# ut-amrl/IV_SLAM

Measured on AMD Instinct MI355X. Metric: stereo pairs/s (extract+match+introspect) @1242×375, 1000 feat; 1/2/4/8 GPU, higher is better.
Workload: dtype u8 (ORB) + f32 via split-f16 MFMA (FCN)

## Files before the change

### iv_slam_amd/csrc/ivf_device.h

```cpp
#pragma once
#include <hip/hip_runtime.h>
#include <stdint.h>
#include <stdlib.h>
#include <vector>
#include "../../include/ivfront.h"

#define DEVINL __device__ __forceinline__

namespace ivf {

constexpr int kMaxLevels = IVF_MAX_LEVELS;
constexpr int kMaxCells = 2048;
constexpr int kEdge = 19;

struct LevelGeom {
    int w, h, pitch;
    int off;
    int nDesired;
    int cols, rows, cellW, cellH, nCells, nfeaturesCell;
    int maxBX, maxBY;
    int domH[2];
    int domHLast;
    int winHLast;
    int cellBase;
    int candBase, candCap;
    int kpBase;
    int scaledPatch;
    int tileBase, tilesX, tilesY;
    int btileBase, btilesX, btilesY;
    int rtX, rtY;
    int valid;
    float scale;
    unsigned cellWMagic, cellHMagic;
};

struct Config {
    int nlevels, w, h;
    int nfeatures, iniTh, minTh, introspection;
    int pyrBytes;
    int candTotal;
    int nCellsTotal;
    int nTiles;
    int nBlurTiles;
    int varBlur, varRetain, varAtan;
    int maxCandCap;
    int umax[16];
    float scale[kMaxLevels], invScale[kMaxLevels];
    int cellBases[kMaxLevels];
    int tileBases[kMaxLevels], btileBases[kMaxLevels];
    LevelGeom lv[kMaxLevels];
};

typedef unsigned long long ResizeCoef;

void resize_axis_table(int ssize, int dsize, int32_t* idx0, int32_t* idx1, int16_t* w0, int16_t* w1);
void resize_axis_pack(int ssize, int dsize, bool columns, bool withIdx1, std::vector<ResizeCoef>& tab);

struct UndistortCam { double fx, fy, cx, cy, k[12]; };
inline UndistortCam undistort_cam(const ivf_camera& c)
{
    UndistortCam u{};
    u.fx = (double)c.fx; u.fy = (double)c.fy; u.cx = (double)c.cx; u.cy = (double)c.cy;
    for (int i = 0; i < 12; i++) u.k[i] = i < c.n_dist ? (double)c.dist[i] : 0.;
    return u;
}
__host__ __device__ inline void undistort_point(const UndistortCam& c, float px, float py, float& ox, float& oy)
{
    const double* k = c.k;
    const double ifx = 1. / c.fx, ify = 1. / c.fy;
    const double u = (double)px, v = (double)py;
    double x = (u - c.cx) * ifx, y = (v - c.cy) * ify;
    const double x0 = x, y0 = y;
    for (int j = 0; j < 5; j++) {
        const double r2 = x * x + y * y;
        const double icdist = (1 + ((k[7] * r2 + k[6]) * r2 + k[5]) * r2) / (1 + ((k[4] * r2 + k[1]) * r2 + k[0]) * r2);
        if (icdist < 0) { x = (u - c.cx) * ifx; y = (v - c.cy) * ify; break; }
        const double dX = 2 * k[2] * x * y + k[3] * (r2 + 2 * x * x) + k[8] * r2 + k[9] * r2 * r2;
        const double dY = k[2] * (r2 + 2 * y * y) + 2 * k[3] * x * y + k[10] * r2 + k[11] * r2 * r2;
        x = (x0 - dX) * icdist; y = (y0 - dY) * icdist;
    }
    const double xx = c.fx * x + 0. * y + c.cx, yy = 0. * x + c.fy * y + c.cy, ww = 1. / (0. * x + 0. * y + 1.);
    ox = (float)(xx * ww); oy = (float)(yy * ww);
}

#ifndef IVF_FAST_TH
#define IVF_FAST_TH 32
#endif
constexpr int kFastTW = 128, kFastTH = IVF_FAST_TH;
constexpr int kBlurTW = 128, kBlurTH = 32;
constexpr int kTileCap = kFastTW * kFastTH / 4;
constexpr int kRowCap = 96;
constexpr int kHugeSlots = 8;
constexpr int kHugeListCap = 4096;

struct CellInfo { int nTotal, nRetain, prefix, useMin; };

struct Buffers {
    uint8_t* pyr;
    uint8_t* qpyr;
    uint8_t* blur;
    unsigned* tileList;
    int* tileCnt;
    int* cellCnt;
    unsigned long long* lvl;
    CellInfo* cellInfo;
    int* lvlTotal;
    unsigned int* slotPos;
    float* slotResp;
    int* lvlCount;
    uint8_t* useCost;
    ivf_keypoint* kps;
    uint8_t* desc;
    int* count;
    float* quality;
    float* uright;
    float* depth;
    int* sad;
    int* rowCnt;
    unsigned short* rowList;
    int* status;
    int* hugeCount;
    int* tierList;
    int* hugeList;
    unsigned* hugeScratch;
};

struct StereoArgs {
    const uint8_t *pyrL, *pyrR; size_t pyrStride;
    const ivf_keypoint *kpL, *kpR; const uint8_t *descL, *descR; const int *cntL, *cntR;
    size_t kpStride;
    int cntStride;
    float *uright, *depth; int* sad; int outStride;
    float bf, bb;
    int* rowCnt; unsigned short* rowList;
};

#ifdef IVF_EXPERIMENT
#define IVF_EXP_ENV(name) getenv(name)
#else
#define IVF_EXP_ENV(name) ((const char*)nullptr)
#endif

void count_launch();
}
#undef hipLaunchKernelGGL
#define hipLaunchKernelGGL(kernelName, ...) do { ivf::count_launch(); hipLaunchKernelGGLInternal((kernelName), __VA_ARGS__); } while (0)
namespace ivf {

int set_error(int code, const char* fmt, ...);

int thread_scratch(int device, size_t need, uint8_t** out);
int thread_pinned(size_t need, uint8_t** out);
int have_device(int dev);

struct BatchImage { const ivf_keypoint *kps, *mvKeys; const uint8_t* desc; const float *uright, *depth, *quality; const int* count; int cap; hipEvent_t done; };
int frame_from_batch(int device, const BatchImage& src, const ivf_bounds& bounds, ivf_frame** out);

void launch_stereo_args(const Config& hc, const Config* dc, const StereoArgs& A, int nPairs, hipStream_t s);
void launch_ingest(const Config& hc, const Config* dc, const uint8_t* src0, const uint8_t* src1, size_t imageStride, int rowStride,
                   int nImg, int nSides, uint8_t* dstBlob, const uint8_t* onlyFlagged, hipStream_t s, int sideMask = 3);
void launch_ingest_color(const Config& hc, const Config* dc, const uint8_t* src, size_t imageStride, int rowStride, int code, int nImg, int nSides, int side,
                         uint8_t* dstBlob, hipStream_t s);
void launch_pyramid(const Config& hc, const Config* dc, const ResizeCoef* dTab, uint8_t* blob, uint8_t* qblob, const uint8_t* useCost,
                    int nImg, hipStream_t s);
void launch_fast(const Config& hc, const Config* dc, const Buffers& b, int nImg, hipStream_t s);
void launch_blur(const Config& hc, const Config* dc, const Buffers& b, int nImg, hipStream_t s, bool skipEmptyLevels);
void launch_describe(const Config& hc, const Config* dc, const Buffers& b, int nImg, hipStream_t s);
void launch_stereo(const Config& hc, const Config* dc, const Buffers& b, int nPairs, float bf, float bb, hipStream_t s);
void launch_pack_gather(const Buffers& b, const ivf_keypoint* kpsUn, int nf, int nPairs, uint8_t* block, size_t recBytes, hipStream_t s);
void launch_select(const Config& hc, const Config* dc, const Buffers& b, int nImg, hipStream_t s);
void launch_test_retain_best(const float* dResp, int n, int nPoints, int* dOrder, unsigned long long* dLists, int* dDiffer, hipStream_t s);
void launch_undistort_keys(const UndistortCam& cam, bool passThrough, const ivf_keypoint* kps, size_t kpStride, const int* count, int cntStride,
                           int nFrames, int cap, ivf_keypoint* out, size_t outStride, hipStream_t s);
// ... 87 lines not shown
```

### iv_slam_amd/csrc/ivf_kernels.hip

```cpp
#include "ivf_grid.h"
#include <cstdlib>

namespace ivf {

static __device__ const int8_t __attribute__((aligned(16))) d_pattern[1024] = {
#include "../../include/ivf_pattern31.inc"
};

DEVINL bool xcd_tile_image(int nTiles, int nImg, int& tile, int& img)
{
    const int xcd = blockIdx.x & 7, j = blockIdx.x >> 3;
    img = (j / nTiles) * 8 + xcd; tile = j % nTiles;
    return img < nImg;
}

constexpr int kIngestRows = 8;
__global__ __launch_bounds__(256) void k_ingest(const Config* __restrict__ cfg, const uint8_t* __restrict__ src0,
                                               const uint8_t* __restrict__ src1, size_t imageStride, int rowStride, int nSides,
                                               uint8_t* __restrict__ blob, const uint8_t* __restrict__ onlyFlagged, int sideMask)
{
    const LevelGeom& G = cfg->lv[0];
    const int img = blockIdx.y, y0 = blockIdx.x * kIngestRows;
    if (onlyFlagged && !(use_cost_of(onlyFlagged, img) & 3u)) return;
    if (!((sideMask >> (img % nSides)) & 1)) return;
// ... 152 lines not shown
        for (int rr = 0; rr < kPyrRPT; rr++) {
            const ResizeCoef c = ty[min(dyFirst + rr, D.h - 1)];
            cyl[rr] = (unsigned)c; cyh[rr] = (unsigned)(c >> 32);
        }
#pragma unroll
        for (int rr = 0; rr < kPyrRPT; rr++) asm volatile("" : "+s"(cyl[rr]), "+s"(cyh[rr]));
#pragma unroll
        for (int rr = 0; rr < kPyrRPT; rr++) {
            const int dy = dyFirst + rr;
            if (dy >= D.h) break;
            const ResizeCoef cy = (ResizeCoef)cyl[rr] | ((ResizeCoef)cyh[rr] << 32);
            const int y0 = (int)(cy & 0xffff), y1 = min(y0 + 1, S.h - 1);
            const unsigned b0 = (unsigned)((cy >> 16) & 0xffff), b1 = (unsigned)((cy >> 32) & 0xffff);
            if (y0 - wy0 == rowB) {
#pragma unroll
                for (int k = 0; k < 4; k++) hA[k] = hB[k];
                rowA = rowB;
            } else if (y0 - wy0 != rowA) { hpass(y0 - wy0, hA); rowA = y0 - wy0; }
            if (y1 - wy0 == rowA) {
#pragma unroll
                for (int k = 0; k < 4; k++) hB[k] = hA[k];
                rowB = rowA;
            } else if (y1 - wy0 != rowB) { hpass(y1 - wy0, hB); rowB = y1 - wy0; }
            unsigned out = 0;
#pragma unroll
            for (int k = 0; k < 4; k++)
                out |= (((__umul24(b0, hA[k]) >> 16) + (__umul24(b1, hB[k]) >> 16) + 2u) >> 2) << (8 * k);
            *(unsigned*)(outp + (size_t)rr * D.pitch) = out & colMask;
        }
        return;
    }
    const int x4 = dx0 + (tid & 63) * 4;
    if (x4 >= D.pitch) return;
    int sxk[4], sx1k[4], a0k[4], a1k[4];
#pragma unroll
    for (int k = 0; k < 4; k++) {
        const int dx = min(x4 + k, D.w - 1);
        const ResizeCoef cx = tx[dx];
        sxk[k] = (int)(cx & 0xffff); sx1k[k] = min(sxk[k] + 1, S.w - 1);
        a0k[k] = (int)((cx >> 16) & 0xffff); a1k[k] = (int)((cx >> 32) & 0xffff);
    }
    for (int rr = 0; rr < kPyrTH / 4; rr++) {
        const int dy = dy0 + (tid >> 6) + 4 * rr;
        if (dy >= D.h) break;
        const ResizeCoef cy = ty[dy];
        const int y0 = (int)(cy & 0xffff), y1 = min(y0 + 1, S.h - 1);
        const int b0 = (int)((cy >> 16) & 0xffff), b1 = (int)((cy >> 32) & 0xffff);
        unsigned out = 0;
#pragma unroll
        for (int k = 0; k < 4; k++) {
            unsigned r = 0;
            if (x4 + k < D.w) {
                int p00, p01, p10, p11;
                const uint8_t* r0 = SP + (size_t)y0 * S.pitch;
                const uint8_t* r1 = SP + (size_t)y1 * S.pitch;
                p00 = r0[sxk[k]]; p01 = r0[sx1k[k]]; p10 = r1[sxk[k]]; p11 = r1[sx1k[k]];
                const int h0 = p00 * a0k[k] + p01 * a1k[k], h1 = p10 * a0k[k] + p11 * a1k[k];
                r = (unsigned)((((b0 * (h0 >> 4)) >> 16) + ((b1 * (h1 >> 4)) >> 16) + 2) >> 2) & 0xffu;
            }
            out |= r << (8 * k);
        }
        *(unsigned*)(base + D.off + (size_t)dy * D.pitch + x4) = out;
    }
}

__global__ __launch_bounds__(256) void k_pyr_down(const Config* __restrict__ cfg, int level, const ResizeCoef* __restrict__ tab,
                                                 uint8_t* __restrict__ blobI, uint8_t* __restrict__ blobQ,
                                                 const uint8_t* __restrict__ useCost, int nImg, int ldsPitch, int ldsRows)
{
    extern __shared__ __attribute__((aligned(16))) uint8_t src[];
    int img = blockIdx.z;
    uint8_t* blob = blobI;
    if (img >= nImg) { img -= nImg; blob = blobQ; if (!(use_cost_of(useCost, img) & 1u)) return; }
    pyr_tile(cfg, level, tab, blob + (size_t)img * cfg->pyrBytes, blockIdx.x * kPyrTW, blockIdx.y * kPyrTH, ldsPitch, ldsRows, src);
}

typedef short s16x2 __attribute__((ext_vector_type(2)));
DEVINL s16x2 pkmin(s16x2 a, s16x2 b) { return __builtin_elementwise_min(a, b); }
DEVINL s16x2 pkmax(s16x2 a, s16x2 b) { return __builtin_elementwise_max(a, b); }
DEVINL s16x2 pair_at(unsigned lo, unsigned hi, int i)
{
    return __builtin_bit_cast(s16x2, __builtin_amdgcn_perm(hi, lo, 0x0c000c00u | ((unsigned)(i + 1) << 16) | (unsigned)i));
}
DEVINL bool compass_test(s16x2 v, s16x2 p0, s16x2 p8, s16x2 p4, s16x2 p12, int t)
{
    const s16x2 T = {(short)t, (short)t};
    const s16x2 X = pkmax(pkmin(p0, p8), pkmin(p4, p12)), Y = pkmin(pkmax(p0, p8), pkmax(p4, p12));
    return ((__builtin_bit_cast(unsigned, X - (v - T)) | __builtin_bit_cast(unsigned, (v + T) - Y)) & 0x80008000u) != 0u;
}
DEVINL bool fast_precheck_pair(unsigned loT, unsigned hiT, unsigned loC, unsigned hiC, unsigned loB, unsigned hiB, int t)
{
    const s16x2 v = pair_at(loC, hiC, 3);
    return compass_test(v, pair_at(loB, hiB, 3), pair_at(loT, hiT, 3), pair_at(loC, hiC, 6), pair_at(loC, hiC, 0), t);
}
DEVINL bool fast_precheck_pair_b(unsigned t0, unsigned t1, unsigned m0, unsigned m1, unsigned m2, unsigned b0, unsigned b1, int t)
{
    const s16x2 v = pair_at(m0, m1, 5);
    return compass_test(v, pair_at(b0, b1, 5), pair_at(t0, t1, 5), pair_at(m1, m2, 4), pair_at(m0, m1, 2), t);
}
DEVINL unsigned fast_score_pair(const unsigned (&lo)[7], const unsigned (&hi)[7], int t)
{
    const s16x2 v = pair_at(lo[3], hi[3], 3);
    s16x2 p[16];
    p[0] = pair_at(lo[6], hi[6], 3);   p[1] = pair_at(lo[6], hi[6], 4);   p[2] = pair_at(lo[5], hi[5], 5);
    p[3] = pair_at(lo[4], hi[4], 6);   p[4] = pair_at(lo[3], hi[3], 6);   p[5] = pair_at(lo[2], hi[2], 6);
    p[6] = pair_at(lo[1], hi[1], 5);   p[7] = pair_at(lo[0], hi[0], 4);   p[8] = pair_at(lo[0], hi[0], 3);
    p[9] = pair_at(lo[0], hi[0], 2);   p[10] = pair_at(lo[1], hi[1], 1);  p[11] = pair_at(lo[2], hi[2], 0);
    p[12] = pair_at(lo[3], hi[3], 0);  p[13] = pair_at(lo[4], hi[4], 0);  p[14] = pair_at(lo[5], hi[5], 1);
    p[15] = pair_at(lo[6], hi[6], 2);
    s16x2 X = pkmin(p[0], p[8]), Y = pkmax(p[0], p[8]);
#pragma unroll
    for (int k = 1; k < 8; k++) { X = pkmax(X, pkmin(p[k], p[k + 8])); Y = pkmin(Y, pkmax(p[k], p[k + 8])); }
    const s16x2 T = {(short)t, (short)t};
    const s16x2 u = X - (v - T), w = (v + T) - Y;
    if (((__builtin_bit_cast(unsigned, u) | __builtin_bit_cast(unsigned, w)) & 0x80008000u) == 0u) return 0u;
    const s16x2 sg = (w >> 15) | (s16x2){1, 1};
    s16x2 q[16];
#pragma unroll
    for (int k = 0; k < 16; k++) q[k] = p[k] * sg;
    s16x2 mx[8];
#pragma unroll
    for (int i = 0; i < 8; i++) { const int j = 2 * i + 1; mx[i] = pkmax(q[j], q[(j + 1) & 15]); }
    s16x2 m4[8];
#pragma unroll
    for (int i = 0; i < 8; i++) m4[i] = pkmax(mx[i], mx[(i + 1) & 7]);
    s16x2 wmin;
#pragma unroll
    for (int i = 0; i < 8; i++) {
        const int j = 2 * i + 1;
        const s16x2 w8 = pkmax(m4[i], m4[(i + 2) & 7]);
        const s16x2 a = pkmax(w8, pkmin(q[(j + 15) & 15], q[(j + 8) & 15]));
        wmin = i ? pkmin(wmin, a) : a;
    }
    const s16x2 amax = v * sg - wmin;
    const int A0 = (int)amax.x, A1 = (int)amax.y;
    const unsigned s0 = A0 > t ? (unsigned)(A0 - 1) : 0u, s1 = A1 > t ? (unsigned)(A1 - 1) : 0u;
    return s0 | (s1 << 16);
}

constexpr int kRawP = kFastTW + 8;
constexpr int kLocalCells = 32;
constexpr int kScW = kFastTW + 2, kScH = kFastTH + 2, kScP = kFastTW + 4;
__global__ __launch_bounds__(256) void k_fast_nms(const Config* __restrict__ cfg, const uint8_t* __restrict__ pyr,
                                                 const uint8_t* __restrict__ useCost, unsigned* __restrict__ tileList,
                                                 int* __restrict__ tileCnt, int* __restrict__ cellCnt, int nImg)
{
    __shared__ __attribute__((aligned(16))) unsigned raw[(kFastTH + 8) * (kRawP / 4) + 4];
    __shared__ __attribute__((aligned(16))) uint8_t sc[(kScH * kScP + 15) / 16 * 16];
    __shared__ unsigned colInfo[kScW + 2], rowInfo[kScH + 2];
    __shared__ int s_cnt[kLocalCells], s_ini[kLocalCells], s_n;
    constexpr int kQuadsA = (kScW + 3) / 4, kRG = 256 / kQuadsA, kRPT = (kScH + kRG - 1) / kRG;
    constexpr int kQRegion = 64 * kRPT * 2;
    static_assert(kRG * kRPT >= kScH && kRG >= 1, "pass A covers the score region");
    __shared__ unsigned s_qmem[4 * kQRegion / 2 > kFastTW * kFastTH / 4 ? 4 * kQRegion / 2 : kFastTW * kFastTH / 4];
    __shared__ int s_nqw[4];
    unsigned short* const s_queue = (unsigned short*)s_qmem;
    unsigned* const s_list = s_qmem;
    constexpr int kCandCap = 32 * kFastTH;
    static_assert(kScW <= 160 && 160 + kScH <= 256, "column classes: threads 0..kScW-1, row classes: threads 160..160+kScH-1");
    __shared__ unsigned short s_cand[kCandCap];
    __shared__ int s_nc;
    int img, bx;
    if (!xcd_tile_image(cfg->nTiles, nImg, bx, img)) return;
    const int tid = threadIdx.x;
    const unsigned useC = use_cost_of(useCost, img);
    int level = 0;
#pragma unroll
    for (int l = 1; l < kMaxLevels; l++) level += bx >= cfg->tileBases[l] ? 1 : 0;
    const LevelGeom G = cfg->lv[level];
    const int t = bx - G.tileBase;
    if (!G.valid || t >= G.tilesX * G.tilesY) { if (tid == 0) tileCnt[(size_t)img * cfg->nTiles + bx] = 0; return; }
    const int tx = t % G.tilesX, ty = t / G.tilesX;
    const int x0 = 16 + tx * kFastTW, y0 = kEdge + ty * kFastTH;
    const uint8_t* src = pyr + (size_t)img * cfg->pyrBytes + G.off;

    constexpr int kRawQ = kRawP / 4, kRawRPP = 256 / kRawQ, kRawIt = (kFastTH + 8 + kRawRPP - 1) / kRawRPP;
    const int rawQ = tid % kRawQ, rawR = tid / kRawQ;
    unsigned rv_[kRawIt];
    {
        const __amdgpu_buffer_rsrc_t rs = __builtin_amdgcn_make_buffer_rsrc((void*)src, 0, G.pitch * G.h, 0x00020000);
        const int gx = x0 - 4 + 4 * rawQ;
        unsigned off = (rawR < kRawRPP && gx < G.pitch) ? (unsigned)((y0 - 4 + rawR) * G.pitch + gx) : 0x7fffffffu;
        const unsigned step = (unsigned)(kRawRPP * G.pitch);
#pragma unroll
        for (int k = 0; k < kRawIt; k++) {
            rv_[k] = __builtin_amdgcn_raw_buffer_load_b32(rs, (int)off, 0, 0);
            off += step;
        }
    }
    for (int i = tid; i < (int)(sizeof(sc) / 16); i += 256) ((uint4*)sc)[i] = make_uint4(0u, 0u, 0u, 0u);
    const int mode = (cfg->introspection && (useC & 1u)) ? 1 : 0;
    const int domHm = mode ? G.domH[1] : G.domH[0];
    if (tid < kScW) {
        const int x = x0 - 1 + tid;
        unsigned f = 0;
        if (x >= kEdge && x < G.maxBX) {
            const int j = G.cellW == 1 ? x - kEdge : (int)__umulhi((unsigned)(x - kEdge), G.cellWMagic);
            const int cx0 = kEdge + j * G.cellW, cx1 = (j == G.cols - 1) ? G.maxBX : cx0 + G.cellW;
            if (x < cx1) f = 1u | ((x - 1 >= cx0) ? 2u : 0u) | ((x + 1 < cx1) ? 4u : 0u) | ((unsigned)j << 8);
        }
        colInfo[tid] = f;
        if (tid < 2) colInfo[kScW + tid] = 0;
    } else if (tid >= 160 && tid < 160 + kScH) {
        const int y = y0 - 1 + (tid - 160);
        unsigned f = 0;
        if (y >= kEdge && y < G.maxBY) {
            int i = G.cellH == 1 ? y - kEdge : (int)__umulhi((unsigned)(y - kEdge), G.cellHMagic);
            if (i > G.rows - 1) i = G.rows - 1;
            const int cy0 = kEdge + i * G.cellH, cy1 = cy0 + ((i == G.rows - 1) ? G.domHLast : domHm);
            if (y < cy1) f = 1u | ((y - 1 >= cy0) ? 2u : 0u) | ((y + 1 < cy1) ? 4u : 0u) | ((unsigned)i << 8);
        }
        rowInfo[tid - 160] = f;
    }
#pragma unroll
    for (int k = 0; k < kRawIt; k++)
        if (rawR < kRawRPP && rawR + kRawRPP * k < kFastTH + 8) raw[(rawR + kRawRPP * k) * kRawQ + rawQ] = rv_[k];
    __syncthreads();
    const int minTh = cfg->minTh;
    constexpr int kQuads = (kScW + 3) / 4;
    if (tid == 0) s_nc = 0;
    {
        const int q = tid % kQuads, rg = tid / kQuads, sx = 4 * q, sy0 = rg * kRPT;
        const bool thr = rg < kRG;
        const int wv = __builtin_amdgcn_readfirstlane(tid >> 6);
        unsigned short* const myq = s_queue + wv * kQRegion;
        const bool cA = thr && ((colInfo[sx] | colInfo[sx + 1]) & 1u), cB = thr && ((colInfo[sx + 2] | colInfo[sx + 3]) & 1u);
        unsigned w0[kRPT + 6], w1[kRPT + 6], w2[kRPT + 6];
#pragma unroll
        for (int j = 0; j < kRPT + 6; j++) {
            const unsigned* base = raw + min(sy0 + j, kFastTH + 7) * (kRawP / 4) + q;
            w0[j] = base[0]; w1[j] = base[1];
            w2[j] = (j >= 3 && j < kRPT + 3) ? base[2] : 0u;
        }
        unsigned rvv[kRPT];
#pragma unroll
        for (int k = 0; k < kRPT; k++) rvv[k] = rowInfo[min(sy0 + k, kScH - 1)];
        int nw = 0;
        const int lane = tid & 63;
#pragma unroll
        for (int k = 0; k < kRPT; k++) {
            const int sy = sy0 + k;
            const bool in = thr && sy < kScH, rowOk = in && (rvv[k] & 1u);
            bool pA = false, pB = false;
            if (rowOk && cA) pA = fast_precheck_pair(w0[k], w1[k], w0[k + 3], w1[k + 3], w0[k + 6], w1[k + 6], minTh);
            if (rowOk && cB) pB = fast_precheck_pair_b(w0[k], w1[k], w0[k + 3], w1[k + 3], w2[k + 3], w0[k + 6], w1[k + 6], minTh);
            const unsigned long long mA = __ballot(pA), mB = __ballot(pB);
            const int nA = __popcll(mA);
            if (pA) myq[nw + (int)__builtin_amdgcn_mbcnt_hi((unsigned)(mA >> 32), __builtin_amdgcn_mbcnt_lo((unsigned)mA, 0u))] = (unsigned short)((sy << 8) | sx);
            if (pB) myq[nw + nA + (int)__builtin_amdgcn_mbcnt_hi((unsigned)(mB >> 32), __builtin_amdgcn_mbcnt_lo((unsigned)mB, 0u))] = (unsigned short)((sy << 8) | (sx + 2));
            nw += nA + __popcll(mB);
        }
        if (lane == 0) s_nqw[wv] = nw;
    }
    __syncthreads();
    const int nq0 = s_nqw[0], nq1 = nq0 + s_nqw[1], nq2 = nq1 + s_nqw[2], nq = nq2 + s_nqw[3];
    for (int i = tid; i < nq; i += 256) {
        const int qi = i < nq0 ? i : (i < nq1 ? kQRegion + i - nq0 : (i < nq2 ? 2 * kQRegion + i - nq1 : 3 * kQRegion + i - nq2));
        const unsigned qe = s_queue[qi];
        const int sy = qe >> 8, sx = qe & 0xff;
        unsigned lo[7], hi[7];
        const int sh = sx & 2;
        const unsigned* base = raw + (sy * kRawP + (sx & ~3)) / 4;
#pragma unroll
        for (int r = 0; r < 7; r++) {
            const unsigned w0 = base[r * (kRawP / 4)], w1 = base[r * (kRawP / 4) + 1], w2 = (r == 0 || r == 6) ? w1 : base[r * (kRawP / 4) + 2];
            lo[r] = __builtin_amdgcn_alignbyte(w1, w0, sh);
            hi[r] = __builtin_amdgcn_alignbyte(w2, w1, sh);
        }
        unsigned two = fast_score_pair(lo, hi, minTh);
        if (!(colInfo[sx] & 1u)) two &= 0xffff0000u;
        if (!(colInfo[sx + 1] & 1u)) two &= 0x0000ffffu;
        const unsigned packed = (two & 0xffu) | ((two >> 8) & 0xff00u);
        *(unsigned short*)(sc + sy * kScP + sx) = (unsigned short)packed;
        const bool rowIn = sy >= 1 && sy <= kFastTH;
        const bool cA = rowIn && (packed & 0xffu) && sx >= 1 && sx <= kFastTW;
        const bool cB = rowIn && (packed >> 8) && sx + 1 <= kFastTW;
        const unsigned long long mA = __ballot(cA), mB = __ballot(cB);
        if (mA | mB) {
            const int lane = tid & 63, lead = __ffsll((long long)(mA | mB)) - 1;
            const int nA = __popcll(mA);
            int qb = 0;
            if (lane == lead) qb = atomicAdd(&s_nc, nA + __popcll(mB));
            qb = __shfl(qb, lead, 64);
            const unsigned long long lt = (1ull << lane) - 1ull;
            const int iA = qb + __popcll(mA & lt), iB = qb + nA + __popcll(mB & lt);
            if (cA && iA < kCandCap) s_cand[iA] = (unsigned short)((sy << 8) | sx);
            if (cB && iB < kCandCap) s_cand[iB] = (unsigned short)((sy << 8) | (sx + 1));
        }
    }
    __syncthreads();
    const int iniTh = cfg->iniTh;
    if (tid < kLocalCells) { s_cnt[tid] = 0; s_ini[tid] = 0; }
    if (tid == 0) s_n = 0;
    const int firstCol = (int)(colInfo[x0 - 1 < kEdge ? kEdge - (x0 - 1) : 1] >> 8);
    int fr = 0;
    for (int q = 1; q <= kFastTH; q++) if (rowInfo[q] & 1u) { fr = (int)(rowInfo[q] >> 8); break; }
    const int firstRow = fr;
    int* cnt = cellCnt + (size_t)img * cfg->nCellsTotal * 2;
    __syncthreads();
    auto nms_one = [&](int sy, int sx, int s) {
        const uint8_t* c = sc + sy * kScP + sx;
        const unsigned ci = colInfo[sx], ri = rowInfo[sy];
        if (!(ci & ri & 1u)) return;
        const int mL = -(int)((ci >> 1) & 1u), mR = -(int)((ci >> 2) & 1u), mU = -(int)((ri >> 1) & 1u), mD = -(int)((ri >> 2) & 1u);
        const int up = max(max((int)c[-kScP - 1] & mL, (int)c[-kScP]), (int)c[-kScP + 1] & mR) & mU;
        const int dn = max(max((int)c[kScP - 1] & mL, (int)c[kScP]), (int)c[kScP + 1] & mR) & mD;
        if (!(s > max(max(up, dn), max((int)c[-1] & mL, (int)c[1] & mR)))) return;
        const int crow = (int)(ri >> 8), ccol = (int)(ci >> 8);
        const int lr = crow - firstRow, lc = ccol - firstCol;
        const int pos = atomicAdd(&s_n, 1);
        if (pos < kTileCap) s_list[pos] = ((unsigned)(y0 + sy - 1) << 20) | ((unsigned)(x0 + sx - 1) << 8) | (unsigned)s;
        if (lr >= 0 && lr < kLocalCells / 4 && lc >= 0 && lc < 4) {
            atomicAdd(&s_cnt[lr * 4 + lc], 1);
            if (s >= iniTh) atomicAdd(&s_ini[lr * 4 + lc], 1);
        } else {
            const int gc = G.cellBase + crow * G.cols + ccol;
            atomicAdd(&cnt[2 * gc], 1);
            if (s >= iniTh) atomicAdd(&cnt[2 * gc + 1], 1);
        }
    };
    const int nc = s_nc;
    if (nc <= kCandCap) {
        for (int i = tid; i < nc; i += 256) {
            const int sy = s_cand[i] >> 8, sx = s_cand[i] & 0xff;
            nms_one(sy, sx, sc[sy * kScP + sx]);
        }
    } else {
        for (int i = tid; i < kFastTH * (kFastTW / 4 + 1); i += 256) {
            const int oy = i / (kFastTW / 4 + 1), q = i % (kFastTW / 4 + 1);
            const unsigned four = *(const unsigned*)(sc + (oy + 1) * kScP + 4 * q);
            if (four == 0) continue;
#pragma unroll
            for (int k = 0; k < 4; k++) {
                const int sx = 4 * q + k;
                const int s = (four >> (8 * k)) & 0xff;
                if (s == 0 || sx < 1 || sx > kFastTW) continue;
                nms_one(oy + 1, sx, s);
            }
        }
    }
    __syncthreads();
    if (tid < kLocalCells && s_cnt[tid] > 0) {
        const int gc = G.cellBase + (firstRow + tid / 4) * G.cols + firstCol + (tid & 3);
        atomicAdd(&cnt[2 * gc], s_cnt[tid]);
        if (s_ini[tid]) atomicAdd(&cnt[2 * gc + 1], s_ini[tid]);
    }
    const int n = s_n;
    unsigned* out = tileList + ((size_t)img * cfg->nTiles + bx) * kTileCap;
    for (int i = tid; i < min(n, kTileCap); i += 256) out[i] = s_list[i];
    if (tid == 0) tileCnt[(size_t)img * cfg->nTiles + bx] = n;
}

DEVINL int reflect101(int p, int n)
{
    if (n == 1) return 0;
    while (p < 0 || p >= n) p = p < 0 ? -p : 2 * (n - 1) - p;
    return p;
}
DEVINL unsigned mad_u16_lo(unsigned a, unsigned k, unsigned c)
{ unsigned r; asm("v_mad_u32_u16 %0, %1, %2, %3" : "=v"(r) : "v"(a), "v"(k), "v"(c)); return r; }
DEVINL unsigned mad_u16_hi(unsigned a, unsigned k, unsigned c)
{ unsigned r; asm("v_mad_u32_u16 %0, %1, %2, %3 op_sel:[1,0,0,0]" : "=v"(r) : "v"(a), "v"(k), "v"(c)); return r; }
__global__ __launch_bounds__(256) void k_blur7(const Config* __restrict__ cfg, const uint8_t* __restrict__ pyr,
                                              const int* __restrict__ lvlCount, uint8_t* __restrict__ blur, int nImg)
{
    constexpr int RQ = (kBlurTW + 8) / 4, RH = kBlurTH + 6, HQ = kBlurTW / 4;
    static_assert(RH % 2 == 0 && HQ == 32 && kBlurTH == 32, "row pairs, 32 quads x 8 row groups");
    __shared__ unsigned raw[RH * RQ];
    __shared__ __attribute__((aligned(16))) uint4 hp[(RH / 2) * HQ];
    int img, bx;
    if (!xcd_tile_image(cfg->nBlurTiles, nImg, bx, img)) return;
    int level = 0;
#pragma unroll
    for (int l = 1; l < kMaxLevels; l++) level += bx >= cfg->btileBases[l] ? 1 : 0;
    const LevelGeom& G = cfg->lv[level];
    const int tilesX = G.btilesX, tilesY = G.btilesY;
    const int t = bx - G.btileBase;
    if (t >= tilesX * tilesY) return;
    if (lvlCount && lvlCount[img * kMaxLevels + level] == 0) return;
    const int x0 = (t % tilesX) * kBlurTW, y0 = (t / tilesX) * kBlurTH;
    const uint8_t* src = pyr + (size_t)img * cfg->pyrBytes + G.off;
    const int tid = threadIdx.x;
    const int gw = G.w, gh = G.h, pitch = G.pitch;
    if (gw >= 8 && gh >= 8) {
        constexpr int RPP = 256 / RQ, IT = (RH + RPP - 1) / RPP;
        const int rq = tid % RQ, r0 = tid / RQ;
        const int gx = x0 - 4 + 4 * rq;
        unsigned v[IT];
        if (x0 - 4 >= 0 && x0 + kBlurTW + 4 <= gw) {
            const __amdgpu_buffer_rsrc_t rs = __builtin_amdgcn_make_buffer_rsrc((void*)src, 0, pitch * gh, 0x00020000);
#pragma unroll
            for (int k = 0; k < IT; k++) {
                const int ry = min(r0 + RPP * k, RH - 1);
                int gy = y0 - 3 + ry; gy = gy < 0 ? -gy : gy; gy = gy >= gh ? 2 * (gh - 1) - gy : gy; gy = max(gy, 0);
                v[k] = __builtin_amdgcn_raw_buffer_load_b32(rs, gy * pitch + gx, 0, 0);
            }
        } else {
            int xb[4];
#pragma unroll
// ... 712 lines not shown
```

### iv_slam_amd/csrc/ivf_select.hip

```cpp
#include "ivf_device.h"
#include <algorithm>

namespace ivf {

typedef unsigned long long u64;
#define RGT(a, b) ((unsigned)((a) >> 32) > (unsigned)((b) >> 32))

template <typename PTR>
DEVINL void sel_adjust_heap(PTR f, int hole, int len, u64 value)
{
    const int top = hole;
    int child = hole;
    while (child < (len - 1) / 2) {
        child = 2 * (child + 1);
        if (RGT(f[child], f[child - 1])) child--;
        f[hole] = f[child];
        hole = child;
    }
    if ((len & 1) == 0 && child == (len - 2) / 2) {
        child = 2 * (child + 1);
        f[hole] = f[child - 1];
        hole = child - 1;
    }
    int parent = (hole - 1) / 2;
// ... 158 lines not shown
    const int wy0 = y0 - 3, wy1 = wy0 + ((i == rows - 1) ? G.winHLast : G.cellH + 6);
    const int a0 = wx0 & ~3, nq = (wx1 - a0 + 3) / 4, nrow = wy1 - wy0;
    unsigned acc = 0;
    constexpr int U = 8;
    const int total = nq * nrow;
    const int dr = 64 / nq, dq = 64 % nq;
    int rr = lane / nq, qq = lane % nq;
    for (int t0 = lane; t0 < total; t0 += 64 * U) {
        unsigned v[U]; int bxs[U];
#pragma unroll
        for (int u = 0; u < U; u++) {
            const bool in = t0 + 64 * u < total;
            const int r = in ? rr : nrow - 1, q = in ? qq : nq - 1;
            bxs[u] = a0 + 4 * q;
            v[u] = *(const unsigned*)(Q + (size_t)(wy0 + r) * G.pitch + bxs[u]);
            qq += dq; rr += dr;
            if (qq >= nq) { qq -= nq; rr++; }
        }
#pragma unroll
        for (int u = 0; u < U; u++) asm volatile("" : "+v"(v[u]));
#pragma unroll
        for (int u = 0; u < U; u++) {
            unsigned w = v[u];
            const int bx = bxs[u];
            if (bx < wx0) w &= 0xffffffffu << (8 * (wx0 - bx));
            if (bx + 4 > wx1) w &= 0xffffffffu >> (8 * (bx + 4 - wx1));
            if (t0 + 64 * u < total) acc = __builtin_amdgcn_sad_u8(w, 0u, acc);
        }
    }
    const unsigned qs = (unsigned)wave_sum_i32((int)acc);
    if (lane == 0) cellInfo[(size_t)img * cfg->nCellsTotal + cell].nTotal = (int)qs;
}

constexpr int kCellCapTiny = 256, kCellCapSmall = 1024, kCellCapBig = 4096;
__global__ __launch_bounds__(256) void k_quota(const Config* __restrict__ cfg, const int* __restrict__ cellCnt,
                                              const uint8_t* __restrict__ qpyr, const uint8_t* __restrict__ useCost,
                                              CellInfo* __restrict__ cellInfo, int* __restrict__ lvlTotal,
                                              int* __restrict__ hugeCount, int* __restrict__ hugeList, int* __restrict__ tierList,
                                              int tierCap, int* __restrict__ status, int cap)
{
    extern __shared__ __attribute__((aligned(16))) int s_quota[];
    int* const s_nIni = s_quota; int* const s_nMin = s_nIni + cap; int* const s_nTotal = s_nMin + cap; int* const s_nRetain = s_nTotal + cap;
    int* const s_prefix = s_nRetain + cap;
    unsigned* const s_qsum = (unsigned*)(s_prefix + cap + 4);
    float* const s_diff = (float*)(s_qsum + cap);
    unsigned char* const s_useMin = (unsigned char*)(s_diff + cap);
    __shared__ float s_wsum;
    const int img = blockIdx.y, level = blockIdx.x;
    const LevelGeom& G = cfg->lv[level];
    const int tid = threadIdx.x;
    if (!G.valid) { if (tid == 0) lvlTotal[img * kMaxLevels + level] = 0; return; }
    const int mode = (cfg->introspection && (use_cost_of(useCost, img) & 1)) ? 1 : 0;
    const int nCells = G.nCells, cols = G.cols, rows = G.rows;
    const int* cnt = cellCnt + ((size_t)img * cfg->nCellsTotal + G.cellBase) * 2;
    CellInfo* ci = cellInfo + (size_t)img * cfg->nCellsTotal + G.cellBase;
    if (mode && G.winHLast <= 0) {
        for (int c = tid; c < nCells; c += 256) ci[c] = CellInfo{0, 0, 0, 0};
        if (tid == 0) lvlTotal[img * kMaxLevels + level] = 0;
        return;
    }
    for (int c = tid; c < nCells; c += 256) {
        s_nMin[c] = cnt[2 * c]; s_nIni[c] = cnt[2 * c + 1];
        s_qsum[c] = mode ? (unsigned)ci[c].nTotal : 0u;
    }
    __syncthreads();
    if (mode) {
        for (int c = tid; c < nCells; c += 256) {
            const int i = c / cols, j = c % cols;
            const float hX = (j == cols - 1) ? (float)(G.maxBX + 3 - (16 + j * G.cellW)) : (float)(G.cellW + 6);
            const float hY = (i == rows - 1) ? (float)G.winHLast : (float)(G.cellH + 6);
            const float cost = (float)s_qsum[c] / (float)(hX * hY);
            const float q = (float)(1.0 / (1.0 + (double)(cost / 255)));
            s_qsum[c] = __float_as_uint(2 * q - 1);
        }
        __syncthreads();
        if (tid == 0) { float wsum = 0.0f; for (int c = 0; c < nCells; c++) wsum += __uint_as_float(s_qsum[c]); s_wsum = wsum; }
        __syncthreads();
    }
    {
        const float wsum = mode ? s_wsum : 1.0f;
        for (int c = tid; c < nCells; c += 256) {
            const float nfc = mode ? fmaxf(1.0f, ceilf((float)G.nDesired * __uint_as_float(s_qsum[c]) / wsum))
                                   : (float)G.nfeaturesCell;
            const bool useMin = s_nIni[c] <= 3;
            const int nKeys = useMin ? s_nMin[c] : s_nIni[c];
            s_useMin[c] = useMin;
            s_nTotal[c] = nKeys;
            if ((float)nKeys > nfc) { s_nRetain[c] = (int)nfc; s_prefix[c] = 0; }
            else { s_nRetain[c] = nKeys; s_diff[c] = nfc - (float)nKeys; s_prefix[c] = 1; }
            s_nIni[c] = __float_as_int(nfc);
        }
    }
    __syncthreads();
    if (tid == 0) {
        int nToDistribute = 0, nNoMore = 0;
        for (int c = 0; c < nCells; c++)
            if (s_prefix[c]) { nToDistribute = (int)((float)nToDistribute + s_diff[c]); nNoMore++; }
        if (nToDistribute > 0 && nNoMore < nCells) {
            for (int c = 0; c < nCells; c++) {
                if (!s_prefix[c]) {
                    const int nNew = (int)(__int_as_float(s_nIni[c]) + ceilf((float)nToDistribute / (nCells - nNoMore)));
                    if (s_nTotal[c] > nNew) s_nRetain[c] = nNew;
                    else { s_nRetain[c] = s_nTotal[c]; nToDistribute += nNew - s_nTotal[c]; s_prefix[c] = 1; nNoMore++; }
                }
            }
        }
        int acc = 0;
        for (int c = 0; c < nCells; c++) {
            const int nT = s_nTotal[c], nR = s_nRetain[c];
            s_prefix[c] = acc;
            acc += (nR >= 0 && nT > nR) ? nR : nT;
        }
        lvlTotal[img * kMaxLevels + level] = acc;
    }
    __syncthreads();
    for (int c = tid; c < nCells; c += 256) {
        ci[c] = CellInfo{s_nTotal[c], s_nRetain[c], s_prefix[c], (int)s_useMin[c]};
        if (s_nTotal[c] > kCellCapTiny && s_nTotal[c] <= kCellCapBig) {
            const int tier = s_nTotal[c] > kCellCapSmall ? 1 : 0;
            const int k = atomicAdd(hugeCount + 1 + tier, 1);
            if (k < tierCap) tierList[(size_t)tier * tierCap + k] = img * cfg->nCellsTotal + G.cellBase + c;
            else atomicOr(status, 4);
        }
        if (s_nTotal[c] > kCellCapBig) {
            const int k = atomicAdd(hugeCount, 1);
            if (hugeList && k < kHugeListCap) hugeList[k] = img * cfg->nCellsTotal + G.cellBase + c;
            else atomicOr(status, 4);
        }
    }
}

constexpr int kSelRows = 512;
struct SelCounts {
    int row[kSelRows + 2];
    int m;
};
template <int CAP>
struct __attribute__((aligned(16))) SelShared {
    static constexpr bool kGlobal = false;
    static constexpr int kCap = CAP;
    typedef unsigned short Stop;
    typedef SyncLds WaveSync;
    unsigned keys[CAP];
    u64 ord[CAP];
    SelCounts c;
};
struct SelGlobal {
    static constexpr bool kGlobal = true;
    typedef unsigned Stop;
    typedef SyncGlobal WaveSync;
    unsigned* keys;
    u64* ord;
    SelCounts& c;
    int cap;
};
template <int NTHR, typename WAVESYNC>
DEVINL void sel_sync()
{
    if constexpr (NTHR == 64) WAVESYNC()(); else __syncthreads();
}
template <int NTHR, typename STORE>
DEVINL void cell_select_one(const Config* __restrict__ cfg, const unsigned* __restrict__ tileList,
                            const int* __restrict__ tileCnt, const CellInfo* __restrict__ cellInfo,
                            const uint8_t* __restrict__ qpyr, const uint8_t* __restrict__ useCost,
                            u64* __restrict__ lvlList, int* __restrict__ status, int nLo, int nHi, int img, int gc, int tid, STORE& S)
{
    typedef typename STORE::Stop Stop;
// ... 307 lines not shown
```

Baseline: 11800.

## Split FAST candidates by threshold and skip low-threshold scoring in ini-rich cells

The FAST precheck now tests each pixel against both the min and ini thresholds and queues high and low candidates in separate regions. High-threshold candidates are scored first and their NMS maxima are counted per local cell. Low-threshold candidates are then scored only for cells whose ini count does not exceed the useMin cutoff (3), because selection ignores min-threshold keys in those cells. This skips full FAST scoring for many weak candidates, at the cost of a second scoring round, extra barriers, and a possible change in which keypoints are emitted at cell boundaries.

```diff
diff --git a/iv_slam_amd/csrc/ivf_device.h b/iv_slam_amd/csrc/ivf_device.h
--- a/iv_slam_amd/csrc/ivf_device.h
+++ b/iv_slam_amd/csrc/ivf_device.h
@@ -89,6 +89,7 @@
 constexpr int kFastTW = 128, kFastTH = IVF_FAST_TH;
 constexpr int kBlurTW = 128, kBlurTH = 32;
 constexpr int kTileCap = kFastTW * kFastTH / 4;
+constexpr int kIniKeepAbove = 3;
 constexpr int kRowCap = 96;
 constexpr int kHugeSlots = 8;
 constexpr int kHugeListCap = 4096;
diff --git a/iv_slam_amd/csrc/ivf_kernels.hip b/iv_slam_amd/csrc/ivf_kernels.hip
--- a/iv_slam_amd/csrc/ivf_kernels.hip
+++ b/iv_slam_amd/csrc/ivf_kernels.hip
@@ -258,21 +258,23 @@
 {
     return __builtin_bit_cast(s16x2, __builtin_amdgcn_perm(hi, lo, 0x0c000c00u | ((unsigned)(i + 1) << 16) | (unsigned)i));
 }
-DEVINL bool compass_test(s16x2 v, s16x2 p0, s16x2 p8, s16x2 p4, s16x2 p12, int t)
-{
-    const s16x2 T = {(short)t, (short)t};
+DEVINL unsigned compass_test2(s16x2 v, s16x2 p0, s16x2 p8, s16x2 p4, s16x2 p12, int tLo, int tHi)
+{
+    const s16x2 TL = {(short)tLo, (short)tLo}, TH = {(short)tHi, (short)tHi};
     const s16x2 X = pkmax(pkmin(p0, p8), pkmin(p4, p12)), Y = pkmin(pkmax(p0, p8), pkmax(p4, p12));
-    return ((__builtin_bit_cast(unsigned, X - (v - T)) | __builtin_bit_cast(unsigned, (v + T) - Y)) & 0x80008000u) != 0u;
-}
-DEVINL bool fast_precheck_pair(unsigned loT, unsigned hiT, unsigned loC, unsigned hiC, unsigned loB, unsigned hiB, int t)
+    const unsigned lo = (__builtin_bit_cast(unsigned, X - (v - TL)) | __builtin_bit_cast(unsigned, (v + TL) - Y)) & 0x80008000u;
+    const unsigned hi = (__builtin_bit_cast(unsigned, X - (v - TH)) | __builtin_bit_cast(unsigned, (v + TH) - Y)) & 0x80008000u;
+    return (lo ? 1u : 0u) | (hi ? 2u : 0u);
+}
+DEVINL unsigned fast_precheck_pair(unsigned loT, unsigned hiT, unsigned loC, unsigned hiC, unsigned loB, unsigned hiB, int tLo, int tHi)
 {
     const s16x2 v = pair_at(loC, hiC, 3);
-    return compass_test(v, pair_at(loB, hiB, 3), pair_at(loT, hiT, 3), pair_at(loC, hiC, 6), pair_at(loC, hiC, 0), t);
-}
-DEVINL bool fast_precheck_pair_b(unsigned t0, unsigned t1, unsigned m0, unsigned m1, unsigned m2, unsigned b0, unsigned b1, int t)
+    return compass_test2(v, pair_at(loB, hiB, 3), pair_at(loT, hiT, 3), pair_at(loC, hiC, 6), pair_at(loC, hiC, 0), tLo, tHi);
+}
+DEVINL unsigned fast_precheck_pair_b(unsigned t0, unsigned t1, unsigned m0, unsigned m1, unsigned m2, unsigned b0, unsigned b1, int tLo, int tHi)
 {
     const s16x2 v = pair_at(m0, m1, 5);
-    return compass_test(v, pair_at(b0, b1, 5), pair_at(t0, t1, 5), pair_at(m1, m2, 4), pair_at(m0, m1, 2), t);
+    return compass_test2(v, pair_at(b0, b1, 5), pair_at(t0, t1, 5), pair_at(m1, m2, 4), pair_at(m0, m1, 2), tLo, tHi);
 }
 DEVINL unsigned fast_score_pair(const unsigned (&lo)[7], const unsigned (&hi)[7], int t)
 {
@@ -392,9 +394,15 @@
     for (int k = 0; k < kRawIt; k++)
         if (rawR < kRawRPP && rawR + kRawRPP * k < kFastTH + 8) raw[(rawR + kRawRPP * k) * kRawQ + rawQ] = rv_[k];
     __syncthreads();
-    const int minTh = cfg->minTh;
+    const int minTh = cfg->minTh, iniTh = cfg->iniTh;
+    const int hiTh = max(iniTh, minTh);
     constexpr int kQuads = (kScW + 3) / 4;
-    if (tid == 0) s_nc = 0;
+    if (tid == 0) { s_nc = 0; s_n = 0; }
+    if (tid < kLocalCells) { s_cnt[tid] = 0; s_ini[tid] = 0; }
+    const int firstCol = (int)(colInfo[x0 - 1 < kEdge ? kEdge - (x0 - 1) : 1] >> 8);
+    int fr = 0;
+    for (int q = 1; q <= kFastTH; q++) if (rowInfo[q] & 1u) { fr = (int)(rowInfo[q] >> 8); break; }
+    const int firstRow = fr;
     {
         const int q = tid % kQuads, rg = tid / kQuads, sx = 4 * q, sy0 = rg * kRPT;
         const bool thr = rg < kRG;
@@ -411,28 +419,82 @@
         unsigned rvv[kRPT];
 #pragma unroll
         for (int k = 0; k < kRPT; k++) rvv[k] = rowInfo[min(sy0 + k, kScH - 1)];
-        int nw = 0;
+        int nwH = 0, nwL = 0;
         const int lane = tid & 63;
+        auto rank_of = [](unsigned long long m) { return (int)__builtin_amdgcn_mbcnt_hi((unsigned)(m >> 32), __builtin_amdgcn_mbcnt_lo((unsigned)m, 0u)); };
 #pragma unroll
         for (int k = 0; k < kRPT; k++) {
             const int sy = sy0 + k;
             const bool in = thr && sy < kScH, rowOk = in && (rvv[k] & 1u);
-            bool pA = false, pB = false;
-            if (rowOk && cA) pA = fast_precheck_pair(w0[k], w1[k], w0[k + 3], w1[k + 3], w0[k + 6], w1[k + 6], minTh);
-            if (rowOk && cB) pB = fast_precheck_pair_b(w0[k], w1[k], w0[k + 3], w1[k + 3], w2[k + 3], w0[k + 6], w1[k + 6], minTh);
-            const unsigned long long mA = __ballot(pA), mB = __ballot(pB);
-            const int nA = __popcll(mA);
-            if (pA) myq[nw + (int)__builtin_amdgcn_mbcnt_hi((unsigned)(mA >> 32), __builtin_amdgcn_mbcnt_lo((unsigned)mA, 0u))] = (unsigned short)((sy << 8) | sx);
-            if (pB) myq[nw + nA + (int)__builtin_amdgcn_mbcnt_hi((unsigned)(mB >> 32), __builtin_amdgcn_mbcnt_lo((unsigned)mB, 0u))] = (unsigned short)((sy << 8) | (sx + 2));
-            nw += nA + __popcll(mB);
-        }
-        if (lane == 0) s_nqw[wv] = nw;
-    }
-    __syncthreads();
-    const int nq0 = s_nqw[0], nq1 = nq0 + s_nqw[1], nq2 = nq1 + s_nqw[2], nq = nq2 + s_nqw[3];
+            unsigned pA = 0u, pB = 0u;
+            if (rowOk && cA) pA = fast_precheck_pair(w0[k], w1[k], w0[k + 3], w1[k + 3], w0[k + 6], w1[k + 6], minTh, hiTh);
+            if (rowOk && cB) pB = fast_precheck_pair_b(w0[k], w1[k], w0[k + 3], w1[k + 3], w2[k + 3], w0[k + 6], w1[k + 6], minTh, hiTh);
+            const unsigned long long hA = __ballot(pA == 3u), hB = __ballot(pB == 3u), lA = __ballot(pA == 1u), lB = __ballot(pB == 1u);
+            const int nhA = __popcll(hA), nlA = __popcll(lA);
+            if (pA == 3u) myq[nwH + rank_of(hA)] = (unsigned short)((sy << 8) | sx);
+            if (pB == 3u) myq[nwH + nhA + rank_of(hB)] = (unsigned short)((sy << 8) | (sx + 2));
+            if (pA == 1u) myq[kQRegion - 1 - (nwL + rank_of(lA))] = (unsigned short)((sy << 8) | sx);
+            if (pB == 1u) myq[kQRegion - 1 - (nwL + nlA + rank_of(lB))] = (unsigned short)((sy << 8) | (sx + 2));
+            nwH += nhA + __popcll(hB);
+            nwL += nlA + __popcll(lB);
+        }
+        if (lane == 0) s_nqw[wv] = nwH | (nwL << 16);
+    }
+    __syncthreads();
+    auto is_max = [&](int sy, int sx, int s, unsigned ci, unsigned ri) {
+        const uint8_t* c = sc + sy * kScP + sx;
+        const int mL = -(int)((ci >> 1) & 1u), mR = -(int)((ci >> 2) & 1u), mU = -(int)((ri >> 1) & 1u), mD = -(int)((ri >> 2) & 1u);
+        const int up = max(max((int)c[-kScP - 1] & mL, (int)c[-kScP]), (int)c[-kScP + 1] & mR) & mU;
+        const int dn = max(max((int)c[kScP - 1] & mL, (int)c[kScP]), (int)c[kScP + 1] & mR) & mD;
+        return s > max(max(up, dn), max((int)c[-1] & mL, (int)c[1] & mR));
+    };
+    auto local_cell = [&](unsigned ci, unsigned ri) {
+        const int lr = (int)(ri >> 8) - firstRow, lc = (int)(ci >> 8) - firstCol;
+        return (lr >= 0 && lr < kLocalCells / 4 && lc >= 0 && lc < 4) ? lr * 4 + lc : -1;
+    };
+    bool iniCounted = false;
+    for (int round = 0; round < 2; round++) {
+    if (round) {
+        const int ncH = s_nc;
+        iniCounted = ncH <= kCandCap;
+        if (iniCounted)
+            for (int i = tid; i < ncH; i += 256) {
+                const int sy = s_cand[i] >> 8, sx = s_cand[i] & 0xff, s = sc[sy * kScP + sx];
+                const unsigned ci = colInfo[sx], ri = rowInfo[sy];
+                const int lc = local_cell(ci, ri);
+                if (s >= iniTh && (ci & ri & 1u) && lc >= 0 && is_max(sy, sx, s, ci, ri)) atomicAdd(&s_ini[lc], 1);
+            }
+        __syncthreads();
+        const int wv = __builtin_amdgcn_readfirstlane(tid >> 6), lane = tid & 63;
+        unsigned short* const myq = s_queue + wv * kQRegion;
+        const int nL = s_nqw[wv] >> 16;
+        int kept = 0;
+        for (int j0 = 0; j0 < nL; j0 += 64) {
+            const int j = j0 + lane;
+            bool need = false;
+            unsigned short qe = 0;
+            if (j < nL) {
+                qe = myq[kQRegion - 1 - j];
+                const int sy = qe >> 8, sx = qe & 0xff;
+                const unsigned ri = rowInfo[sy], c0 = colInfo[sx], c1 = colInfo[sx + 1];
+                auto needed = [&](unsigned ci) {
+                    if (!(ci & ri & 1u)) return false;
+                    const int lc = local_cell(ci, ri);
+                    return !(iniCounted && lc >= 0 && s_ini[lc] > kIniKeepAbove);
+                };
+                need = needed(c0) || needed(c1);
+            }
+            const unsigned long long m = __ballot(need);
+            if (need) myq[kQRegion - 1 - (kept + __popcll(m & ((1ull << lane) - 1ull)))] = qe;
+            kept += __popcll(m);
+        }
+        if (lane == 0) s_nqw[wv] = kept;
+        __syncthreads();
+    }
+    const int nq0 = s_nqw[0] & 0xffff, nq1 = nq0 + (s_nqw[1] & 0xffff), nq2 = nq1 + (s_nqw[2] & 0xffff), nq = nq2 + (s_nqw[3] & 0xffff);
     for (int i = tid; i < nq; i += 256) {
-        const int qi = i < nq0 ? i : (i < nq1 ? kQRegion + i - nq0 : (i < nq2 ? 2 * kQRegion + i - nq1 : 3 * kQRegion + i - nq2));
-        const unsigned qe = s_queue[qi];
+        const int wq = i < nq0 ? 0 : (i < nq1 ? 1 : (i < nq2 ? 2 : 3)), j = i - (wq == 0 ? 0 : (wq == 1 ? nq0 : (wq == 2 ? nq1 : nq2)));
+        const unsigned qe = s_queue[wq * kQRegion + (round ? kQRegion - 1 - j : j)];
         const int sy = qe >> 8, sx = qe & 0xff;
         unsigned lo[7], hi[7];
         const int sh = sx & 2;
@@ -465,32 +527,22 @@
         }
     }
     __syncthreads();
-    const int iniTh = cfg->iniTh;
-    if (tid < kLocalCells) { s_cnt[tid] = 0; s_ini[tid] = 0; }
-    if (tid == 0) s_n = 0;
-    const int firstCol = (int)(colInfo[x0 - 1 < kEdge ? kEdge - (x0 - 1) : 1] >> 8);
-    int fr = 0;
-    for (int q = 1; q <= kFastTH; q++) if (rowInfo[q] & 1u) { fr = (int)(rowInfo[q] >> 8); break; }
-    const int firstRow = fr;
+    }
     int* cnt = cellCnt + (size_t)img * cfg->nCellsTotal * 2;
-    __syncthreads();
     auto nms_one = [&](int sy, int sx, int s) {
-        const uint8_t* c = sc + sy * kScP + sx;
         const unsigned ci = colInfo[sx], ri = rowInfo[sy];
         if (!(ci & ri & 1u)) return;
-        const int mL = -(int)((ci >> 1) & 1u), mR = -(int)((ci >> 2) & 1u), mU = -(int)((ri >> 1) & 1u), mD = -(int)((ri >> 2) & 1u);
-        const int up = max(max((int)c[-kScP - 1] & mL, (int)c[-kScP]), (int)c[-kScP + 1] & mR) & mU;
-        const int dn = max(max((int)c[kScP - 1] & mL, (int)c[kScP]), (int)c[kScP + 1] & mR) & mD;
-        if (!(s > max(max(up, dn), max((int)c[-1] & mL, (int)c[1] & mR)))) return;
-        const int crow = (int)(ri >> 8), ccol = (int)(ci >> 8);
-        const int lr = crow - firstRow, lc = ccol - firstCol;
+        if (!is_max(sy, sx, s, ci, ri)) return;
+        const int l = local_cell(ci, ri);
+        const bool flagged = iniCounted && l >= 0 && s_ini[l] > kIniKeepAbove;
+        if (s < iniTh && flagged) return;
         const int pos = atomicAdd(&s_n, 1);
         if (pos < kTileCap) s_list[pos] = ((unsigned)(y0 + sy - 1) << 20) | ((unsigned)(x0 + sx - 1) << 8) | (unsigned)s;
-        if (lr >= 0 && lr < kLocalCells / 4 && lc >= 0 && lc < 4) {
-            atomicAdd(&s_cnt[lr * 4 + lc], 1);
-            if (s >= iniTh) atomicAdd(&s_ini[lr * 4 + lc], 1);
+        if (l >= 0) {
+            atomicAdd(&s_cnt[l], 1);
+            if (!iniCounted && s >= iniTh) atomicAdd(&s_ini[l], 1);
         } else {
-            const int gc = G.cellBase + crow * G.cols + ccol;
+            const int gc = G.cellBase + (int)(ri >> 8) * G.cols + (int)(ci >> 8);
             atomicAdd(&cnt[2 * gc], 1);
             if (s >= iniTh) atomicAdd(&cnt[2 * gc + 1], 1);
         }
diff --git a/iv_slam_amd/csrc/ivf_select.hip b/iv_slam_amd/csrc/ivf_select.hip
--- a/iv_slam_amd/csrc/ivf_select.hip
+++ b/iv_slam_amd/csrc/ivf_select.hip
@@ -264,7 +264,7 @@
         for (int c = tid; c < nCells; c += 256) {
             const float nfc = mode ? fmaxf(1.0f, ceilf((float)G.nDesired * __uint_as_float(s_qsum[c]) / wsum))
                                    : (float)G.nfeaturesCell;
-            const bool useMin = s_nIni[c] <= 3;
+            const bool useMin = s_nIni[c] <= kIniKeepAbove;
             const int nKeys = useMin ? s_nMin[c] : s_nIni[c];
             s_useMin[c] = useMin;
             s_nTotal[c] = nKeys;
```

New measurement: 11710. No clear change (-0.7%).
